# telespazio-tim/karios

Measured on AMD Instinct MI355X. Metric: Mpixels/sec (+ matched keypoints/sec), Sentinel-2 10980^2 pair, KLT + ZNCC, higher is better.
Workload: dtype u8/i32 stencils, f32 LK solve, f64 stretch + ZNCC; 1 GPU; BASELINE config 2: 4 distinct S2-sized pairs 10980x10980 u16 resident in HBM, one per step, 4 per batched submissio...; distinct_pairs_resident=4, contexts=1, klt=Laplacian k=7, maxCorners 20000, one tile, ZNCC of rows with score >= 0.4, parallelism=1 rank(s), each a stream of independent band pairs

## Files before the change

karios_amd/csrc/k_lap.hip:

```cpp
#include "k_pixel.hpp"
#include "lap_coef.hpp"

#include <algorithm>

#ifndef KM_LAPM_WAVES
#define KM_LAPM_WAVES 0
#endif
#if KM_LAPM_WAVES
#define KM_LAPM_OCC __attribute__((amdgpu_waves_per_eu(KM_LAPM_WAVES, KM_LAPM_WAVES)))
#else
#define KM_LAPM_OCC
#endif

#define LAP_TW 128
#define LAP_TH 16

template <typename T> struct stretcher {
    double mn, range;
    bool deg;
    __device__ void init(const double *mm, int img, const uint8_t *) {
        if constexpr (sizeof(T) == 1) { mn = 0; range = 1; deg = false; }
        else { mn = mm[2 * img]; const double mx = mm[2 * img + 1]; range = mx - mn; deg = !(mx > mn); }
    }
    __device__ __forceinline__ unsigned operator()(T v, const uint8_t *) const { return stretch_u8<T>(v, mn, range, deg); }
};
template <typename T> struct stretcher_i16 {
    int mn_i;
    double c1, c0;
    __device__ void init(const double *mm, int img, const uint8_t *) {
        const double mn = mm[2 * img], mx = mm[2 * img + 1];
        mn_i = (int)mn;
        if (mx > mn) { const double r = mx - mn; c1 = 255.0 / r; c0 = 0.5 / r; }
        else { c1 = 0.0; c0 = 0.0; }
    }
    __device__ __forceinline__ unsigned operator()(T v, const uint8_t *) const {
        return (unsigned)(int)__fma_rn((double)((int)v - mn_i), c1, c0);
    }
};
template <> struct stretcher<uint16_t> : stretcher_i16<uint16_t> {};
template <> struct stretcher<int16_t> : stretcher_i16<int16_t> {};

template <int R, typename T, int NIMG, bool MASK>
__global__ __launch_bounds__(256) void lap_kernel(const T *__restrict__ img0, const T *__restrict__ img1, int H, int W,
                                                  ptrdiff_t stride0, ptrdiff_t stride1, const double *__restrict__ mm,
                                                  lap_coef cf, int invert1, nodata_t nd,
                                                  uint8_t *__restrict__ out0, uint8_t *__restrict__ out1,
                                                  uint8_t *__restrict__ mask_out, unsigned *__restrict__ valid_partial)
{
    using HT = typename std::conditional<(R <= 3), short, int>::type;
    constexpr int HX = (R + 3) & ~3;
    constexpr int TWH = LAP_TW + 2 * HX;
    constexpr int THH = LAP_TH + 2 * R;
    constexpr int CPR = TWH / 4;
    constexpr int NQ = LAP_TW / 4;
    constexpr int NIT = (THH * CPR + 255) / 256;
    __shared__ uint32_t tile[NIMG][THH][CPR];
    __shared__ __attribute__((aligned(16))) HT hbuf[2][NIMG][THH][LAP_TW];
    auto &hd = hbuf[0];
    auto &hs = hbuf[1];
    const int X0 = blockIdx.x * LAP_TW, Y0 = blockIdx.y * LAP_TH;
    const int tid = threadIdx.x;
    stretcher<T> st[NIMG];
#pragma unroll
    for (int i = 0; i < NIMG; i++) st[i].init(mm, i, nullptr);
    const T *imgs[2] = {img0, img1};
    const ptrdiff_t strides[2] = {stride0, stride1};

    T v[NIT][NIMG][4];
#pragma unroll
    for (int it = 0; it < NIT; it++) {
        const int ci = it * 256 + tid;
        if (ci < THH * CPR) {
            const int row = ci / CPR, cx = ci - row * CPR;
            const int gy = km_reflect101(Y0 - R + row, H);
            const int gx0 = X0 - HX + cx * 4;
            const bool inside = gx0 >= 0 && gx0 + 3 < W;
#pragma unroll
            for (int i = 0; i < NIMG; i++) {
                const T *rowp = imgs[i] + (size_t)gy * strides[i];
                if (inside && ((((uintptr_t)(rowp + gx0)) & (4 * sizeof(T) - 1)) == 0)) {
                    if constexpr (sizeof(T) == 1) { uint32_t q = *(const uint32_t *)(rowp + gx0); __builtin_memcpy(v[it][i], &q, 4); }
                    else if constexpr (sizeof(T) == 2) { uint2 q = *(const uint2 *)(rowp + gx0); __builtin_memcpy(v[it][i], &q, 8); }
                    else { uint4 q = *(const uint4 *)(rowp + gx0); __builtin_memcpy(v[it][i], &q, 16); }
                } else {
#pragma unroll
                    for (int k = 0; k < 4; k++) v[it][i][k] = rowp[km_reflect101(gx0 + k, W)];
                }
            }
        }
    }
    unsigned cnt = 0;
#pragma unroll
    for (int it = 0; it < NIT; it++) {
        const int ci = it * 256 + tid;
        if (ci < THH * CPR) {
            const int row = ci / CPR, cx = ci - row * CPR;
            const int gx0 = X0 - HX + cx * 4;
#pragma unroll
            for (int i = 0; i < NIMG; i++) {
                uint32_t packed = 0;
#pragma unroll
                for (int k = 0; k < 4; k++) {
                    unsigned u = st[i](v[it][i][k], nullptr);
                    if (i == 1 && invert1) u = 255u - u;
                    packed |= u << (8 * k);
                }
                tile[i][row][cx] = packed;
            }
            if constexpr (MASK) {
                const int oy = Y0 - R + row;
                if (row >= R && row < R + LAP_TH && oy < H && gx0 >= X0 && gx0 < X0 + LAP_TW && gx0 < W) {
                    uint32_t mp = 0;
#pragma unroll
                    for (int k = 0; k < 4; k++) {
                        const bool ok = (gx0 + k < W) && px_valid<T>(v[it][1][k], v[it][0][k], nd);
                        mp |= (ok ? 1u : 0u) << (8 * k);
                        cnt += ok;
                    }
                    const size_t o = (size_t)oy * W + gx0;
                    if (gx0 + 3 < W && (o & 3) == 0) *(uint32_t *)(mask_out + o) = mp;
                    else {
                        for (int k = 0; k < 4 && gx0 + k < W; k++) mask_out[o + k] = (uint8_t)((mp >> (8 * k)) & 1u);
                    }
                }
            }
        }
    }
    if constexpr (MASK) {
        __shared__ unsigned s_cnt[4];
        const unsigned c64 = (unsigned)wave_sum_u64((unsigned long long)cnt);
        if ((tid & 63) == 0) s_cnt[tid >> 6] = c64;
        __syncthreads();
        if (tid == 0) valid_partial[blockIdx.y * gridDim.x + blockIdx.x] = s_cnt[0] + s_cnt[1] + s_cnt[2] + s_cnt[3];
    } else {
        __syncthreads();
    }

    uint8_t *outs[2] = {out0, out1};
    if constexpr (R <= 3) {
        typedef short short2v __attribute__((ext_vector_type(2)));
        int *hds = (int *)&hd[0][0][0];
        int kdp[NIMG][2], ksp[NIMG][2], bias[NIMG], vk[NIMG][2 * R + 1];
#pragma unroll
        for (int i = 0; i < NIMG; i++) {
            int sum = 0;
#pragma unroll
            for (int h = 0; h < 2; h++) {
                unsigned a = 0, b = 0;
#pragma unroll
                for (int k = 0; k < 4; k++) {
                    const int t = 4 * h + k;
                    const int d = t <= 2 * R ? cf.kd[i][t] : 0, sm = t <= 2 * R ? cf.ks[i][t] : 0;
                    a |= ((unsigned)d & 0xffu) << (8 * k);
                    b |= ((unsigned)sm & 0xffu) << (8 * k);
                    sum += sm;
                }
                kdp[i][h] = (int)a; ksp[i][h] = (int)b;
            }
            bias[i] = R == 4 ? 0 : 128 * sum;
#pragma unroll
            for (int t = 0; t <= 2 * R; t++) vk[i][t] = (cf.ks[i][t] & 0xffff) | (cf.kd[i][t] << 16);
        }
        for (int it = tid; it < NIMG * THH * NQ; it += 256) {
            const int i = it / (THH * NQ);
            const int rem = it - i * (THH * NQ);
            const int row = rem / NQ, q = rem - row * NQ;
            uint32_t w[4];
#pragma unroll
            for (int k = 0; k < 4; k++) w[k] = ((q + k < CPR) ? tile[i][row][q + k] : 0u) ^ 0x80808080u;
            int o4[4];
#pragma unroll
            for (int o = 0; o < 4; o++) {
                constexpr int base = HX - R;
                const int sft = (o + base) & 3, wi = (o + base) >> 2;
                const int g0 = (int)__builtin_amdgcn_alignbyte(w[wi + 1], w[wi], sft);
                const int g1 = (int)__builtin_amdgcn_alignbyte(wi + 2 < 4 ? w[wi + 2] : 0u, w[wi + 1], sft);
                const int vd = __builtin_amdgcn_sdot4(g0, kdp[i][0], __builtin_amdgcn_sdot4(g1, kdp[i][1], 0, false), false);
                const int vs = __builtin_amdgcn_sdot4(g0, ksp[i][0], __builtin_amdgcn_sdot4(g1, ksp[i][1], bias[i], false), false);
                o4[o] = (vd & 0xffff) | (vs << 16);
            }
            *(int4 *)&hds[((size_t)i * THH + row) * LAP_TW + 4 * q] = make_int4(o4[0], o4[1], o4[2], o4[3]);
        }
        __syncthreads();
        for (int it = tid; it < NIMG * (LAP_TH / 4) * NQ; it += 256) {
            const int i = it / ((LAP_TH / 4) * NQ);
            const int rem = it - i * ((LAP_TH / 4) * NQ);
            const int rg = rem / NQ, q = rem - rg * NQ;
            const int ox = X0 + 4 * q;
            if (ox >= W || Y0 + 4 * rg >= H) continue;
            int acc[4][4];
#pragma unroll
            for (int o = 0; o < 4; o++)
#pragma unroll
                for (int c2 = 0; c2 < 4; c2++) acc[o][c2] = 0;
#pragma unroll
            for (int j = 0; j < 2 * R + 4; j++) {
                const int4 a = *(const int4 *)&hds[((size_t)i * THH + 4 * rg + j) * LAP_TW + 4 * q];
                const int av[4] = {a.x, a.y, a.z, a.w};
#pragma unroll
                for (int o = 0; o < 4; o++) {
                    const int tap = j - o;
                    if (tap >= 0 && tap <= 2 * R) {
#pragma unroll
                        for (int c2 = 0; c2 < 4; c2++)
                            acc[o][c2] = __builtin_amdgcn_sdot2(__builtin_bit_cast(short2v, av[c2]), __builtin_bit_cast(short2v, vk[i][tap]),
                                                                acc[o][c2], false);
                    }
                }
            }
#pragma unroll
            for (int o = 0; o < 4; o++) {
                const int oy = Y0 + 4 * rg + o;
                if (oy >= H) break;
                uint32_t packed = 0;
#pragma unroll
                for (int k = 0; k < 4; k++) packed |= (uint32_t)min(max(acc[o][k], 0), 255) << (8 * k);
                const size_t off = (size_t)oy * W + ox;
                if (ox + 3 < W && (off & 3) == 0) *(uint32_t *)(outs[i] + off) = packed;
                else {
                    for (int k = 0; k < 4 && ox + k < W; k++) outs[i][off + k] = (uint8_t)(packed >> (8 * k));
                }
            }
        }
    } else {
        constexpr int NW = (2 * R + 4 + (HX - R) + 3) / 4;
        for (int it = tid; it < NIMG * THH * NQ; it += 256) {
            const int i = it / (THH * NQ);
            const int rem = it - i * (THH * NQ);
            const int row = rem / NQ, q = rem - row * NQ;
            uint32_t w[NW + 1];
#pragma unroll
            for (int k = 0; k < NW + 1; k++) w[k] = (q + k < CPR) ? tile[i][row][q + k] : 0u;
            int ad[4] = {0, 0, 0, 0}, as[4] = {0, 0, 0, 0};
#pragma unroll
            for (int t = 0; t < 2 * R + 4; t++) {
                const int b = t + (HX - R);
                const int pv = (int)((w[b >> 2] >> (8 * (b & 3))) & 0xffu);
#pragma unroll
                for (int o = 0; o < 4; o++) {
                    const int k = t - o;
                    if (k >= 0 && k <= 2 * R) {
                        ad[o] = mad24(cf.kd[i][k], pv, ad[o]);
                        as[o] = mad24(cf.ks[i][k], pv, as[o]);
                    }
                }
            }
            HT *pd = &hd[i][row][4 * q], *ps = &hs[i][row][4 * q];
#pragma unroll
            for (int o = 0; o < 4; o++) { pd[o] = (HT)ad[o]; ps[o] = (HT)as[o]; }
        }
        __syncthreads();
        for (int it = tid; it < NIMG * (LAP_TH / 4) * NQ; it += 256) {
            const int i = it / ((LAP_TH / 4) * NQ);
            const int rem = it - i * ((LAP_TH / 4) * NQ);
            const int rg = rem / NQ, q = rem - rg * NQ;
            const int ox = X0 + 4 * q;
            if (ox >= W || Y0 + 4 * rg >= H) continue;
            int acc[4][4];
#pragma unroll
            for (int o = 0; o < 4; o++)
#pragma unroll
                for (int c2 = 0; c2 < 4; c2++) acc[o][c2] = 0;
#pragma unroll
            for (int j = 0; j < 2 * R + 4; j++) {
                const HT *pa = &hd[i][4 * rg + j][4 * q], *pb = &hs[i][4 * rg + j][4 * q];
                int a[4], b[4];
#pragma unroll
                for (int c2 = 0; c2 < 4; c2++) { a[c2] = pa[c2]; b[c2] = pb[c2]; }
#pragma unroll
                for (int o = 0; o < 4; o++) {
                    const int tap = j - o;
                    if (tap >= 0 && tap <= 2 * R) {
                        const int ksj = cf.ks[i][tap], kdj = cf.kd[i][tap];
#pragma unroll
                        for (int c2 = 0; c2 < 4; c2++) acc[o][c2] = mad24(ksj, a[c2], mad24(kdj, b[c2], acc[o][c2]));
                    }
                }
            }
#pragma unroll
            for (int o = 0; o < 4; o++) {
                const int oy = Y0 + 4 * rg + o;
                if (oy >= H) break;
                uint32_t packed = 0;
#pragma unroll
                for (int k = 0; k < 4; k++) packed |= (uint32_t)min(max(acc[o][k], 0), 255) << (8 * k);
                const size_t off = (size_t)oy * W + ox;
                if (ox + 3 < W && (off & 3) == 0) *(uint32_t *)(outs[i] + off) = packed;
                else {
                    for (int k = 0; k < 4 && ox + k < W; k++) outs[i][off + k] = (uint8_t)(packed >> (8 * k));
                }
            }
        }
    }
}

template <typename T, int NIMG, bool MASK>
static int launch_lap(km_ctx *c, int R, const T *a, const T *b, int H, int W, ptrdiff_t sa, ptrdiff_t sb, const double *mm,
                      const lap_coef &cf, int invert1, const nodata_t &nd, uint8_t *oa, uint8_t *ob, uint8_t *mask,
                      unsigned long long *valid_out)
{
    dim3 grid((W + LAP_TW - 1) / LAP_TW, (H + LAP_TH - 1) / LAP_TH);
    unsigned *valid = nullptr;
    if (MASK) {
        valid = (unsigned *)km_ws(c, WS_PARTIAL, (size_t)grid.x * grid.y * sizeof(unsigned));
        if (!valid) return KM_E_NOMEM;
    }
#define KM_LAP_CASE(RR)                                                                                         \
    case RR:                                                                                                    \
        lap_kernel<RR, T, NIMG, MASK><<<grid, 256, 0, c->stream>>>(a, b, H, W, sa, sb, mm, cf, invert1, nd, oa, ob, \
                                                                   mask, valid);                               \
        break;
    switch (R) {
        KM_LAP_CASE(1)
        KM_LAP_CASE(2)
        KM_LAP_CASE(3)
        KM_LAP_CASE(4)
        KM_LAP_CASE(5)
    default: return km_fail(c, KM_E_UNSUPPORTED, "laplacian radius %d", R);
    }
#undef KM_LAP_CASE
    KM_LAUNCH_CHECK(c);
    return MASK ? kd_sum_u32(c, valid, grid.x * grid.y, valid_out) : KM_OK;
}

__device__ __forceinline__ int dot4_seed0(int bytes, int coef_uniform)
{
    int r;
    asm("v_dot4_i32_i8 %0, %1, %2, 0" : "=v"(r) : "v"(bytes), "s"(coef_uniform));
    return r;
}
__device__ __forceinline__ int dot4_seed(int bytes, int coef_uniform, int acc)
{
    int r;
    asm("v_dot4_i32_i8 %0, %1, %2, %3" : "=v"(r) : "v"(bytes), "s"(coef_uniform), "v"(acc));
    return r;
}
__device__ __forceinline__ int dot2_seed0(int pair, int coef_uniform)
{
    int r;
    asm("v_dot2_i32_i16 %0, %1, %2, 0" : "=v"(r) : "v"(pair), "s"(coef_uniform));
    return r;
}
__device__ __forceinline__ unsigned opaque_lane_offset(unsigned x)
{
    asm volatile("" : "+v"(x));
    return x;
}

#define LAPM_VALID_OF(R) ((R) == 5 ? 240 : 248)
#ifndef LAPM_PF
#define LAPM_PF 3
#endif

template <int R, typename T, bool MASK>
__device__ __forceinline__ void lap_march_item(const T *__restrict__ img0, const T *__restrict__ img1, int H, int W,
                                               ptrdiff_t stride0, ptrdiff_t stride1, const double *__restrict__ mm,
                                               const lap_coef &cf, int invert1, const nodata_t &nd,
                                               uint8_t *__restrict__ out0, uint8_t *__restrict__ out1,
                                               uint8_t *__restrict__ mask_out, unsigned *__restrict__ valid_partial, int nstrips,
                                               int rows_per_item, int wave_id )
{
    typedef short short2v __attribute__((ext_vector_type(2)));
    constexpr int RH = R == 5 ? 4 : R;
    constexpr int NR = 2 * RH + 1;
    constexpr int HALO = R == 5 ? 8 : 4, VALID = 256 - 2 * HALO;
    static_assert(VALID == LAPM_VALID_OF(R), "strip geometry");
    const int lane = threadIdx.x & 63;
    const int rowblock = wave_id / nstrips, strip = wave_id - rowblock * nstrips;
    stretcher<T> st[2];
    st[0].init(mm, 0, nullptr); st[1].init(mm, 1, nullptr);
    const bool shifted = (W % 4 != 0) && strip == nstrips - 1 && W >= 256;
    const int gx0 = (shifted ? W - (256 - HALO) : strip * VALID - HALO) + 4 * lane;
    const int cnt_from = shifted ? (nstrips - 1) * VALID : 0;
    const uint32_t cnt_mask = gx0 >= cnt_from ? 0xffffffffu : gx0 + 4 <= cnt_from ? 0u : (0xffffffffu << (8 * (cnt_from - gx0)));
    const unsigned ugx = (unsigned)gx0;
    const unsigned ugx_load = RH == 4 ? (unsigned)min(max(gx0 < 0 ? -gx0 - 3 : gx0 >= W ? 2 * W - 5 - gx0 : gx0, 0), W - 4) : (unsigned)min(max(gx0, 0), W - 4);
    const unsigned edge_sel = RH == 4 ? ((gx0 < 0 || gx0 >= W) ? 0x00010203u : 0x03020100u)
                                      : (gx0 < 0 ? 0x01020300u : gx0 >= W ? 0x03000102u : 0x03020100u);
    const bool col_inside = gx0 >= 0 && gx0 + 3 < W;
    const bool vec0 = col_inside && (stride0 % 4 == 0) && ((uintptr_t)img0 % (4 * sizeof(T)) == 0);
    const bool vec1 = col_inside && (stride1 % 4 == 0) && ((uintptr_t)img1 % (4 * sizeof(T)) == 0);
    int rc[4];
#pragma unroll
    for (int k = 0; k < 4; k++) rc[k] = km_reflect101(gx0 + k, W);
    const bool out_lane = lane >= HALO / 4 && lane <= 63 - HALO / 4 && gx0 < W;
    const int y0 = rowblock * rows_per_item, y1 = min(H, y0 + rows_per_item);

    constexpr int NH = RH == 4 ? 3 : 2;
    int kdp[2][NH], ksp[2][NH], bias[2], vk[2][NR];
#pragma unroll
    for (int i = 0; i < 2; i++) {
        int sum = 0;
#pragma unroll
        for (int h = 0; h < NH; h++) {
            unsigned a = 0, b = 0;
#pragma unroll
            for (int k = 0; k < 4; k++) {
                const int t = 4 * h + k;
                const int d = t < NR ? cf.kd[i][t] : 0, sm = t < NR ? cf.ks[i][t] : 0;
                a |= ((unsigned)d & 0xffu) << (8 * k);
                b |= ((unsigned)sm & 0xffu) << (8 * k);
                sum += sm;
            }
            kdp[i][h] = (int)a; ksp[i][h] = (int)b;
        }
        bias[i] = 128 * sum;
#pragma unroll
        for (int t = 0; t < NR; t++) vk[i][t] = (cf.ks[i][t] & 0xffff) | (cf.kd[i][t] << 16);
    }

    typedef unsigned short ushort2v __attribute__((ext_vector_type(2)));
    auto nodata16 = [](int has, double v) -> uint32_t {
        if (!has || v != floor(v)) return 0u;
        if constexpr (std::is_signed<T>::value) { if (v < -32768.0 || v > 32767.0) return 0u; }
        else { if (v < 0.0 || v > 65535.0) return 0u; }
        const uint32_t x = (uint32_t)(uint16_t)(int)v;
        return x | (x << 16);
    };
    const uint32_t nd16_mon = nodata16(nd.has_mon, nd.mon), nd16_ref = nodata16(nd.has_ref, nd.ref);
    (void)nd16_mon; (void)nd16_ref;
    int vbias[2];
    asm volatile("v_mov_b32 %0, %1" : "=v"(vbias[0]) : "s"(bias[0]));
    asm volatile("v_mov_b32 %0, %1" : "=v"(vbias[1]) : "s"(bias[1]));
    unsigned cnt = 0;
    uint8_t *outs[2] = {out0, out1};
    auto march = [&](auto fast_tag) {
    constexpr bool FAST = decltype(fast_tag)::value;
    auto load_raw = [&](int m, T (&v)[2][4]) {
        const int r = km_reflect101(m, H);
        const T *r0 = img0 + (size_t)r * stride0, *r1 = img1 + (size_t)r * stride1;
        const unsigned lx = opaque_lane_offset(ugx_load * (unsigned)sizeof(T));
        if (FAST) {
            __builtin_memcpy(v[0], (const char *)r0 + lx, 4 * sizeof(T));
        } else if (vec0) {
            if constexpr (sizeof(T) == 1) { uint32_t q = *(const uint32_t *)(r0 + gx0); __builtin_memcpy(v[0], &q, 4); }
            else if constexpr (sizeof(T) == 2) { uint2 q = *(const uint2 *)(r0 + gx0); __builtin_memcpy(v[0], &q, 8); }
            else { uint4 q = *(const uint4 *)(r0 + gx0); __builtin_memcpy(v[0], &q, 16); }
        } else {
#pragma unroll
            for (int k = 0; k < 4; k++) v[0][k] = r0[rc[k]];
        }
        if (FAST) {
            __builtin_memcpy(v[1], (const char *)r1 + lx, 4 * sizeof(T));
        } else if (vec1) {
            if constexpr (sizeof(T) == 1) { uint32_t q = *(const uint32_t *)(r1 + gx0); __builtin_memcpy(v[1], &q, 4); }
            else if constexpr (sizeof(T) == 2) { uint2 q = *(const uint2 *)(r1 + gx0); __builtin_memcpy(v[1], &q, 8); }
            else { uint4 q = *(const uint4 *)(r1 + gx0); __builtin_memcpy(v[1], &q, 16); }
        } else {
#pragma unroll
            for (int k = 0; k < 4; k++) v[1][k] = r1[rc[k]];
        }
    };

    int hp[2][2][4];
#pragma unroll
    for (int i = 0; i < 2; i++)
#pragma unroll
        for (int r = 0; r < 2; r++)
#pragma unroll
            for (int j = 0; j < 4; j++) hp[i][r][j] = 0;
    (void)hp;
    int ring[2][NR][4];
#pragma unroll
    for (int i = 0; i < 2; i++)
#pragma unroll
        for (int k = 0; k < NR; k++)
#pragma unroll
            for (int j = 0; j < 4; j++) ring[i][k][j] = 0;
    T nxt[LAPM_PF][2][4];
#pragma unroll
    for (int f = 0; f < LAPM_PF; f++) load_raw(min(y0 - R + f, y1 + R - 1), nxt[f]);
    for (int mbase = y0 - R; mbase < y1 + R; mbase += NR) {
#pragma unroll
        for (int k = 0; k < NR; k++) {
            const int m = mbase + k;
            if (m >= y1 + R) continue;
            T v[2][4];
#pragma unroll
            for (int i = 0; i < 2; i++)
#pragma unroll
                for (int j = 0; j < 4; j++) {
                    v[i][j] = nxt[0][i][j];
#pragma unroll
                    for (int f = 0; f + 1 < LAPM_PF; f++) nxt[f][i][j] = nxt[f + 1][i][j];
                }
            if (m + LAPM_PF < y1 + R) load_raw(m + LAPM_PF, nxt[LAPM_PF - 1]);
            if constexpr (MASK && FAST && sizeof(T) == 2) {
                if (m >= y0 && m < y1 && out_lane) {
                    uint2 qm, qr;
                    __builtin_memcpy(&qm, v[1], 8); __builtin_memcpy(&qr, v[0], 8);
                    auto nz2 = [&](uint32_t a, uint32_t b) {
                        ushort2v mn2 = __builtin_elementwise_min(
                            __builtin_elementwise_min(__builtin_bit_cast(ushort2v, a), __builtin_bit_cast(ushort2v, b)),
                            __builtin_elementwise_min(__builtin_bit_cast(ushort2v, a ^ nd16_mon), __builtin_bit_cast(ushort2v, b ^ nd16_ref)));
                        mn2 = __builtin_elementwise_min(mn2, (ushort2v)(1));
                        return __builtin_bit_cast(uint32_t, mn2);
                    };
                    const uint32_t mp = __builtin_amdgcn_perm(nz2(qm.y, qr.y), nz2(qm.x, qr.x), 0x06040200u);
                    cnt += (unsigned)__popc(mp & cnt_mask);
                    __builtin_memcpy((mask_out + (size_t)m * W) + opaque_lane_offset(ugx), &mp, 4);
                }
            } else if constexpr (MASK) {
                if (m >= y0 && m < y1 && out_lane) {
                    uint32_t mp = 0;
#pragma unroll
                    for (int j = 0; j < 4; j++) {
                        const bool ok = (gx0 + j < W) && px_valid<T>(v[1][j], v[0][j], nd);
                        mp |= (ok ? 1u : 0u) << (8 * j);
                        cnt += ok && gx0 + j >= cnt_from;
                    }
                    const size_t o = (size_t)m * W + gx0;
                    if (FAST) __builtin_memcpy(mask_out + o, &mp, 4);
                    else if (gx0 + 3 < W && (o & 3) == 0) *(uint32_t *)(mask_out + o) = mp;
                    else {
                        for (int j = 0; j < 4 && gx0 + j < W; j++) mask_out[o + j] = (uint8_t)((mp >> (8 * j)) & 1u);
                    }
                }
            }
#pragma unroll
            for (int i = 0; i < 2; i++) {
                uint32_t cw = 0;
#pragma unroll
                for (int j = 0; j < 4; j++) cw |= st[i](v[i][j], nullptr) << (8 * j);
                cw ^= (i == 1 && invert1) ? 0x7f7f7f7fu : 0x80808080u;
                if constexpr (FAST) cw = __builtin_amdgcn_perm(cw, cw, edge_sel);
                const uint32_t lw = (uint32_t)__builtin_amdgcn_update_dpp(0, (int)cw, 0x138, 0xf, 0xf, false);
                const uint32_t rw = (uint32_t)__builtin_amdgcn_update_dpp(0, (int)cw, 0x130, 0xf, 0xf, false);
#pragma unroll
                for (int o = 0; o < 4; o++) {
                    constexpr int dummy = 0; (void)dummy;
                    if constexpr (RH == 4) {
                        const int g0 = (int)__builtin_amdgcn_alignbyte(cw, lw, o), g1 = (int)__builtin_amdgcn_alignbyte(rw, cw, o),
                                  g2 = (int)__builtin_amdgcn_alignbyte(0u, rw, o);
                        const int vd = __builtin_amdgcn_sdot4(g0, kdp[i][0], __builtin_amdgcn_sdot4(g1, kdp[i][1], dot4_seed0(g2, kdp[i][2]), false), false);
                        const int vs = __builtin_amdgcn_sdot4(g0, ksp[i][0], __builtin_amdgcn_sdot4(g1, ksp[i][1], dot4_seed0(g2, ksp[i][2]), false), false);
                        ring[i][k][o] = (int)__builtin_amdgcn_perm((uint32_t)vs, (uint32_t)vd, 0x05040100u);
                        continue;
                    }
                    const int sft = 4 + o - R;
                    int g0, g1;
                    if (sft < 4) {
                        g0 = (int)__builtin_amdgcn_alignbyte(cw, lw, sft & 3);
                        g1 = (int)__builtin_amdgcn_alignbyte(rw, cw, sft & 3);
                    } else if (sft == 4) {
                        g0 = (int)cw; g1 = (int)rw;
                    } else {
                        g0 = (int)__builtin_amdgcn_alignbyte(rw, cw, (sft - 4) & 3);
                        g1 = (int)__builtin_amdgcn_alignbyte(0u, rw, (sft - 4) & 3);
                    }
                    const int vd = __builtin_amdgcn_sdot4(g0, kdp[i][0], dot4_seed0(g1, kdp[i][1]), false);
                    const int vs = __builtin_amdgcn_sdot4(g0, ksp[i][0], dot4_seed(g1, ksp[i][1], vbias[i]), false);
                    ring[i][k][o] = (int)__builtin_amdgcn_perm((uint32_t)vs, (uint32_t)vd, 0x05040100u);
                }
            }
            if constexpr (R == 5) {
                const int yy = m - RH, yo = yy - 1;
                if (yy >= y0 - 1) {
#pragma unroll
                    for (int i = 0; i < 2; i++) {
                        int a[4], h[4];
#pragma unroll
                        for (int o = 0; o < 4; o++) {
                            int acc = dot2_seed0(ring[i][(k + 1) % NR][o], vk[i][0]);
#pragma unroll
                            for (int j = 1; j < NR; j++)
                                acc = __builtin_amdgcn_sdot2(__builtin_bit_cast(short2v, ring[i][(k + 1 + j) % NR][o]),
                                                             __builtin_bit_cast(short2v, vk[i][j]), acc, false);
                            a[o] = acc;
                        }
                        uint32_t packed = 0;
                        if (cf.b3[i]) {
                            const int al = __builtin_amdgcn_update_dpp(0, a[3], 0x138, 0xf, 0xf, false);
                            const int ar = __builtin_amdgcn_update_dpp(0, a[0], 0x130, 0xf, 0xf, false);
#pragma unroll
                            for (int o = 0; o < 4; o++) h[o] = (o == 0 ? al : a[o - 1]) + 2 * a[o] + (o == 3 ? ar : a[o + 1]);
#pragma unroll
                            for (int o = 0; o < 4; o++) packed |= (uint32_t)min(max(hp[i][1][o] + 2 * hp[i][0][o] + h[o], 0), 255) << (8 * o);
                        } else {
#pragma unroll
                            for (int o = 0; o < 4; o++) { h[o] = a[o]; packed |= (uint32_t)min(max(hp[i][0][o], 0), 255) << (8 * o); }
                        }
#pragma unroll
                        for (int o = 0; o < 4; o++) { hp[i][1][o] = hp[i][0][o]; hp[i][0][o] = h[o]; }
                        if (yo >= y0 && out_lane) {
                            const size_t off = (size_t)yo * W + gx0;
                            if (FAST) __builtin_memcpy((outs[i] + (size_t)yo * W) + opaque_lane_offset(ugx), &packed, 4);
                            else if (gx0 + 3 < W && (off & 3) == 0) *(uint32_t *)(outs[i] + off) = packed;
                            else {
                                for (int j = 0; j < 4 && gx0 + j < W; j++) outs[i][off + j] = (uint8_t)(packed >> (8 * j));
                            }
                        }
                    }
                }
            } else {
            const int y = m - R;
            if (y >= y0 && out_lane) {
#pragma unroll
                for (int i = 0; i < 2; i++) {
                    uint32_t packed = 0;
#pragma unroll
                    for (int o = 0; o < 4; o++) {
                        int acc = dot2_seed0(ring[i][(k + 1) % NR][o], vk[i][0]);
#pragma unroll
                        for (int j = 1; j < NR; j++)
                            acc = __builtin_amdgcn_sdot2(__builtin_bit_cast(short2v, ring[i][(k + 1 + j) % NR][o]),
                                                         __builtin_bit_cast(short2v, vk[i][j]), acc, false);
                        packed |= (uint32_t)min(max(acc, 0), 255) << (8 * o);
                    }
                    const size_t off = (size_t)y * W + gx0;
                    if (FAST) __builtin_memcpy((outs[i] + (size_t)y * W) + opaque_lane_offset(ugx), &packed, 4);
                    else if (gx0 + 3 < W && (off & 3) == 0) *(uint32_t *)(outs[i] + off) = packed;
                    else {
                        for (int j = 0; j < 4 && gx0 + j < W; j++) outs[i][off + j] = (uint8_t)(packed >> (8 * j));
                    }
                }
            }
            }
        }
    }
    };
    const bool fast = (W % 4 == 0) || shifted || (strip * VALID - HALO + 4 * 64 <= W);
    if (fast) march(std::true_type{});
    else march(std::false_type{});
    if constexpr (MASK) {
        const unsigned c64 = (unsigned)wave_sum_u64((unsigned long long)cnt);
        if (lane == 0) valid_partial[wave_id] = c64;
    }
}

struct lapm_units_args {
    const void *img0[KM_UNITS_MAX], *img1[KM_UNITS_MAX];
    ptrdiff_t s0[KM_UNITS_MAX], s1[KM_UNITS_MAX];
    const double *mm[KM_UNITS_MAX];
    uint8_t *out0[KM_UNITS_MAX], *out1[KM_UNITS_MAX], *mask[KM_UNITS_MAX];
    unsigned *valid[KM_UNITS_MAX];
    int H[KM_UNITS_MAX], W[KM_UNITS_MAX], nstrips[KM_UNITS_MAX];
    int item0[KM_UNITS_MAX + 1];
    int n, rows;
};
template <int R, typename T, bool MASK>
__global__ __launch_bounds__(256) KM_LAPM_OCC void lap_march_units_kernel(lapm_units_args U, lap_coef cf, int invert1, nodata_t nd)
{
    const int total = U.item0[U.n];
    unsigned tile;
    if (!km_xcd_tile((unsigned)(total + 3) / 4u, tile)) return;
    const int wave_lin = (int)tile * 4 + __builtin_amdgcn_readfirstlane(threadIdx.x >> 6);
    if (wave_lin >= total) return;
    int u = 0;
    while (u + 1 < U.n && wave_lin >= U.item0[u + 1]) u++;
    lap_march_item<R, T, MASK>((const T *)U.img0[u], (const T *)U.img1[u], U.H[u], U.W[u], U.s0[u], U.s1[u], U.mm[u], cf, invert1, nd, U.out0[u], U.out1[u],
                               U.mask[u], U.valid[u], U.nstrips[u], U.rows, wave_lin - U.item0[u]);
}

template <typename T, bool MASK>
static const void *lapm_kernel(int R)
{
    return R == 1 ? (const void *)lap_march_units_kernel<1, T, MASK> : R == 2 ? (const void *)lap_march_units_kernel<2, T, MASK>
         : R == 3 ? (const void *)lap_march_units_kernel<3, T, MASK> : R == 4 ? (const void *)lap_march_units_kernel<4, T, MASK>
         : (const void *)lap_march_units_kernel<5, T, MASK>;
}

static void lapm_items(km_ctx *c, int R, const void *fn, lapm_units_args &A)
{
    int wg_per_cu = 0;
    if (hipOccupancyMaxActiveBlocksPerMultiprocessor(&wg_per_cu, fn, 256, 0) != hipSuccess || wg_per_cu < 1) wg_per_cu = 4;
    int rows = km_pick_rows_units(A.H, A.nstrips, A.n, 2 * R, (long)c->n_cu * 4 * wg_per_cu, 32, 160);
    if (const char *e = km_dev_env("KARIOS_HIP_LAP_ROWS")) { const int v = atoi(e); if (v >= 8 && v <= 4096) rows = v; }
    A.rows = rows;
    A.item0[0] = 0;
    for (int u = 0; u < A.n; u++) A.item0[u + 1] = A.item0[u] + A.nstrips[u] * ((A.H[u] + rows - 1) / rows);
}

static int lapm_launch(km_ctx *c, const void *fn, const lapm_units_args &A, const lap_coef &cf, int invert1, const nodata_t &nd)
{
    void *args[] = {(void *)&A, (void *)&cf, (void *)&invert1, (void *)&nd};
    KM_HIP(c, hipLaunchKernel(fn, dim3(km_xcd_grid((unsigned)(A.item0[A.n] + 3) / 4u)), dim3(256), args, 0, c->stream));
    return KM_OK;
}

template <typename T, bool MASK>
static int launch_lap_march(km_ctx *c, int R, const T *a, const T *b, int H, int W, ptrdiff_t sa, ptrdiff_t sb, const double *mm,
                            const lap_coef &cf, int invert1, const nodata_t &nd, uint8_t *oa, uint8_t *ob,
                            uint8_t *mask, unsigned long long *valid_out, km_valid_job *defer)
{
    lapm_units_args A;
    A.n = 1;
    A.img0[0] = a; A.img1[0] = b; A.s0[0] = sa; A.s1[0] = sb; A.mm[0] = mm;
    A.out0[0] = oa; A.out1[0] = ob; A.mask[0] = mask; A.valid[0] = nullptr;
    A.H[0] = H; A.W[0] = W; A.nstrips[0] = (W + LAPM_VALID_OF(R) - 1) / LAPM_VALID_OF(R);
    const void *fn = lapm_kernel<T, MASK>(R);
    lapm_items(c, R, fn, A);
    const unsigned nitems = (unsigned)A.item0[1];
    if (MASK) {
        A.valid[0] = (unsigned *)km_ws(c, WS_LAP_VALID, ((size_t)nitems + 4) * sizeof(unsigned));
        if (!A.valid[0]) return KM_E_NOMEM;
    }
    if (int rc = lapm_launch(c, fn, A, cf, invert1, nd)) return rc;
    if (MASK) {
        if (defer) {
            defer->partial = A.valid[0]; defer->n = nitems; defer->out = valid_out;
        } else if (int rc = kd_sum_u32(c, A.valid[0], nitems, valid_out)) return rc;
    }
    return KM_OK;
}

int kd_run_valid_sum(km_ctx *c, km_valid_job *job)
{
    if (!job->partial) return KM_OK;
    const km_valid_job j = *job;
    *job = km_valid_job();
    return kd_sum_u32(c, j.partial, j.n, j.out);
}

__global__ __launch_bounds__(64) void valid_sum_units_kernel(km_valid_units J)
{
    const unsigned *partial = J.partial[blockIdx.x];
    const unsigned n = J.n_partial[blockIdx.x];
    unsigned long long s = 0;
    for (unsigned i = threadIdx.x; i < n; i += 64) s += partial[i];
    s = wave_sum_u64(s);
    if (threadIdx.x == 0) *J.out[blockIdx.x] = s;
}

int kd_valid_sum_units(km_ctx *c, const km_valid_units &J)
{
    if (J.n <= 0) return KM_OK;
    valid_sum_units_kernel<<<J.n, 64, 0, c->stream>>>(J);
    KM_LAUNCH_CHECK(c);
    return KM_OK;
}

struct mask_units_args {
    const uint8_t *src[KM_UNITS_MAX];
    uint8_t *dst[KM_UNITS_MAX];
    ptrdiff_t stride[KM_UNITS_MAX];
    unsigned *partial[KM_UNITS_MAX];
    int H[KM_UNITS_MAX], W[KM_UNITS_MAX];
};
__global__ __launch_bounds__(256) void mask_pack_units_kernel(mask_units_args A)
{
    const int u = blockIdx.y, H = A.H[u], W = A.W[u];
    const uint8_t *__restrict__ src = A.src[u];
    uint8_t *__restrict__ dst = A.dst[u];
    const ptrdiff_t stride = A.stride[u];
    unsigned cnt = 0;
    for (int y = blockIdx.x; y < H; y += gridDim.x) {
        const uint8_t *r = src + (size_t)y * stride;
        uint8_t *w = dst + (size_t)y * W;
        for (int x = 16 * threadIdx.x; x < W; x += 16 * 256) {
            if (x + 16 <= W) {
                uint4 q;
                __builtin_memcpy(&q, r + x, 16);
                __builtin_memcpy(w + x, &q, 16);
                const uint32_t d[4] = {q.x, q.y, q.z, q.w};
#pragma unroll
                for (int k = 0; k < 4; k++) cnt += (unsigned)__popc(((d[k] | ((d[k] & 0x7f7f7f7fu) + 0x7f7f7f7fu)) & 0x80808080u));
            } else {
                for (int k = x; k < W; k++) { const uint8_t b = r[k]; w[k] = b; cnt += b != 0; }
            }
        }
    }
    const unsigned long long s = wave_sum_u64((unsigned long long)cnt);
    __shared__ unsigned sh[4];
    if ((threadIdx.x & 63) == 0) sh[threadIdx.x >> 6] = (unsigned)s;
    __syncthreads();
    if (threadIdx.x == 0) A.partial[u][blockIdx.x] = sh[0] + sh[1] + sh[2] + sh[3];
}

template <typename T>
static int launch_lap_march_units(km_ctx *c, int R, const km_units &U, const lap_coef &cf, int invert1, const nodata_t &nd, km_valid_units *job)
{
    lapm_units_args A;
    A.n = U.n;
    for (int u = 0; u < U.n; u++) {
        A.img0[u] = U.ref[u]; A.img1[u] = U.mon[u]; A.s0[u] = U.sref[u]; A.s1[u] = U.smon[u]; A.mm[u] = U.mm[u];
        A.out0[u] = U.lap_ref[u]; A.out1[u] = U.lap_mon[u]; A.mask[u] = U.mask[u];
        A.H[u] = U.H[u]; A.W[u] = U.W[u]; A.nstrips[u] = (U.W[u] + LAPM_VALID_OF(R) - 1) / LAPM_VALID_OF(R);
    }
    lapm_items(c, R, lapm_kernel<T, true>(R), A);
    const int total = A.item0[U.n];
    const int mask_wgs = 256;
    const size_t n_partial = U.has_user_mask ? (size_t)mask_wgs * U.n : (size_t)total + 4 * KM_UNITS_MAX;
    unsigned *valid = (unsigned *)km_ws(c, WS_LAP_VALID, n_partial * sizeof(unsigned));
    if (!valid) return KM_E_NOMEM;
    job->n = U.n;
    if (U.has_user_mask) {
        mask_units_args M;
        for (int u = 0; u < U.n; u++) {
            M.src[u] = U.user_mask[u]; M.dst[u] = U.mask[u]; M.stride[u] = U.user_smask[u]; M.H[u] = U.H[u]; M.W[u] = U.W[u];
            M.partial[u] = valid + (size_t)mask_wgs * u;
            A.valid[u] = nullptr;
            job->partial[u] = M.partial[u]; job->n_partial[u] = (unsigned)mask_wgs; job->out[u] = &U.sc[u]->valid;
        }
        mask_pack_units_kernel<<<dim3(mask_wgs, U.n), 256, 0, c->stream>>>(M);
        KM_LAUNCH_CHECK(c);
        return lapm_launch(c, lapm_kernel<T, false>(R), A, cf, invert1, nd);
    }
    for (int u = 0; u < U.n; u++) {
        A.valid[u] = valid + A.item0[u];
        job->partial[u] = A.valid[u]; job->n_partial[u] = (unsigned)(A.item0[u + 1] - A.item0[u]); job->out[u] = &U.sc[u]->valid;
    }
    return lapm_launch(c, lapm_kernel<T, true>(R), A, cf, invert1, nd);
}

enum lap_form { LAP_NOT_COVERED = 0, LAP_GENERAL, LAP_MARCH };
struct lap_plan {
    int R = 0;
    lap_coef cf;
    lap_form form = LAP_NOT_COVERED;
};
static lap_plan lap_make_plan(int ksize_ref, int ksize_mon, int min_W, int min_H)
{
    lap_plan p;
    if (!km_lap_ksize_ok(ksize_ref) || !km_lap_ksize_ok(ksize_mon)) return p;
    const int ks[2] = {ksize_ref, ksize_mon};
    p.R = std::max(std::max(ksize_ref, ksize_mon) / 2, 1);
    const int edge = p.R == 5 ? 16 : 8;
    const bool march = min_W >= edge && min_H >= edge, march5 = march && p.R == 5;
    for (int i = 0; i < 2; i++) {
        p.cf.b3[i] = march5 && ks[i] == 11;
        if (!fill_coef(p.cf.b3[i] ? 9 : ks[i], march5 ? 4 : p.R, p.cf.kd[i], p.cf.ks[i])) return p;
    }
    p.form = march ? LAP_MARCH : LAP_GENERAL;
    return p;
}

int kd_stretch_laplacian_units(km_ctx *c, const km_units &U, int ksize_ref, int ksize_mon, int invert_mon, const double *nodata_ref,
                               const double *nodata_mon, km_valid_units *job)
{
    const lap_plan p = lap_make_plan(ksize_ref, ksize_mon, *std::min_element(U.W, U.W + U.n), *std::min_element(U.H, U.H + U.n));
    if (p.form == LAP_NOT_COVERED) return km_fail(c, KM_E_UNSUPPORTED, "Laplacian ksize ref=%d mon=%d (supported: 1,3,5,7,9,11)", ksize_ref, ksize_mon);
    if (p.form != LAP_MARCH) return KM_E_UNSUPPORTED;
    const nodata_t nd = make_nodata(nodata_mon, nodata_ref);
    return km_with_pixel_type(c, U.dtype, "stretch_laplacian: bad dtype %d",
                              [&](auto t) { return launch_lap_march_units<decltype(t)>(c, p.R, U, p.cf, invert_mon, nd, job); });
}

int kd_laplacian_u8(km_ctx *c, const uint8_t *d_src, int H, int W, int ksize, uint8_t *d_dst)
{
    const lap_plan p = lap_make_plan(ksize, ksize, 0, 0);
    if (p.form == LAP_NOT_COVERED) return km_fail(c, KM_E_UNSUPPORTED, "Laplacian ksize %d (supported: 1,3,5,7,9,11)", ksize);
    return launch_lap<uint8_t, 1, false>(c, p.R, d_src, d_src, H, W, W, W, nullptr, p.cf, 0, make_nodata(nullptr, nullptr), d_dst, nullptr, nullptr,
                                         nullptr);
}

int kd_stretch_laplacian_pair(km_ctx *c, const void *d_ref, const void *d_mon, int dtype, int H, int W, ptrdiff_t sref,
                              ptrdiff_t smon, const double *d_mm, int ksize_ref, int ksize_mon, int invert_mon,
                              const double *nodata_ref, const double *nodata_mon, uint8_t *d_lap_ref, uint8_t *d_lap_mon,
                              uint8_t *d_mask_out, unsigned long long *d_valid, km_valid_job *defer)
{
    const lap_plan p = lap_make_plan(ksize_ref, ksize_mon, W, H);
    if (p.form == LAP_NOT_COVERED) return km_fail(c, KM_E_UNSUPPORTED, "Laplacian ksize ref=%d mon=%d (supported: 1,3,5,7,9,11)", ksize_ref, ksize_mon);
    const nodata_t nd = make_nodata(nodata_mon, nodata_ref);
    return km_with_pixel_type(c, dtype, "stretch_laplacian: bad dtype %d", [&](auto t) {
        using T = decltype(t);
        const T *ref = (const T *)d_ref, *mon = (const T *)d_mon;
        if (p.form == LAP_MARCH)
            return d_mask_out ? launch_lap_march<T, true>(c, p.R, ref, mon, H, W, sref, smon, d_mm, p.cf, invert_mon, nd, d_lap_ref, d_lap_mon, d_mask_out, d_valid, defer)
                              : launch_lap_march<T, false>(c, p.R, ref, mon, H, W, sref, smon, d_mm, p.cf, invert_mon, nd, d_lap_ref, d_lap_mon, nullptr, nullptr, nullptr);
        return d_mask_out ? launch_lap<T, 2, true>(c, p.R, ref, mon, H, W, sref, smon, d_mm, p.cf, invert_mon, nd, d_lap_ref, d_lap_mon, d_mask_out, d_valid)
                          : launch_lap<T, 2, false>(c, p.R, ref, mon, H, W, sref, smon, d_mm, p.cf, invert_mon, nd, d_lap_ref, d_lap_mon, nullptr, nullptr);
    });
}
```

Before: 153,700 Mpx/s.

## Split Laplacian march into warmup and branch-free interior loop with buffer stores

Restructures the row-march loop of the fused Laplacian/mask kernel into three phases: a guarded warmup, a branch-free interior phase, and a guarded tail. The interior phase uses a rotating slot buffer with pointer-increment loads, raw buffer stores whose out-of-range lanes are handled by the buffer descriptor bounds, and sched barriers between rows. This removes per-row boundary checks and 64-bit address arithmetic from the hot loop. It also swaps update_dpp for mov_dpp with bound_ctrl. The cost is more code and register pressure, plus a risk that the descriptor bounds or lane masking are subtly wrong.

```diff
diff --git a/karios_amd/csrc/k_lap.hip b/karios_amd/csrc/k_lap.hip
--- a/karios_amd/csrc/k_lap.hip
+++ b/karios_amd/csrc/k_lap.hip
@@ -346,6 +346,12 @@
     asm volatile("" : "+v"(x));
     return x;
 }
+__device__ __forceinline__ void reopaque_lane_offset(unsigned &x) { asm volatile("" : "+v"(x)); }
+template <class F, int... I> __device__ __forceinline__ void lapm_for_impl(F &&f, std::integer_sequence<int, I...>)
+{
+    (f(std::integral_constant<int, I>{}), ...);
+}
+template <int N, class F> __device__ __forceinline__ void lapm_for(F &&f) { lapm_for_impl(f, std::make_integer_sequence<int, N>{}); }
 
 #define LAPM_VALID_OF(R) ((R) == 5 ? 240 : 248)
 #ifndef LAPM_PF
@@ -467,26 +473,16 @@
         for (int k = 0; k < NR; k++)
 #pragma unroll
             for (int j = 0; j < 4; j++) ring[i][k][j] = 0;
-    T nxt[LAPM_PF][2][4];
-#pragma unroll
-    for (int f = 0; f < LAPM_PF; f++) load_raw(min(y0 - R + f, y1 + R - 1), nxt[f]);
-    for (int mbase = y0 - R; mbase < y1 + R; mbase += NR) {
-#pragma unroll
-        for (int k = 0; k < NR; k++) {
-            const int m = mbase + k;
-            if (m >= y1 + R) continue;
-            T v[2][4];
-#pragma unroll
-            for (int i = 0; i < 2; i++)
-#pragma unroll
-                for (int j = 0; j < 4; j++) {
-                    v[i][j] = nxt[0][i][j];
-#pragma unroll
-                    for (int f = 0; f + 1 < LAPM_PF; f++) nxt[f][i][j] = nxt[f + 1][i][j];
-                }
-            if (m + LAPM_PF < y1 + R) load_raw(m + LAPM_PF, nxt[LAPM_PF - 1]);
+    __amdgpu_buffer_rsrc_t rs_m = __builtin_amdgcn_make_buffer_rsrc((void *)nullptr, 0, 0, 0x00020000), rs_o0 = rs_m, rs_o1 = rs_m;
+    unsigned srow = 0;
+    const unsigned ux = out_lane ? ugx : 0x80000000u;
+    const uint32_t cnt_mask_in = out_lane ? cnt_mask : 0u;
+    (void)srow; (void)ux; (void)cnt_mask_in;
+    auto row_step = [&](auto k_tag, auto in_tag, int m, const T (&v)[2][4]) {
+            constexpr int k = decltype(k_tag)::value;
+            constexpr bool IN = decltype(in_tag)::value;
             if constexpr (MASK && FAST && sizeof(T) == 2) {
-                if (m >= y0 && m < y1 && out_lane) {
+                if (IN || (m >= y0 && m < y1 && out_lane)) {
                     uint2 qm, qr;
                     __builtin_memcpy(&qm, v[1], 8); __builtin_memcpy(&qr, v[0], 8);
                     auto nz2 = [&](uint32_t a, uint32_t b) {
@@ -497,20 +493,29 @@
                         return __builtin_bit_cast(uint32_t, mn2);
                     };
                     const uint32_t mp = __builtin_amdgcn_perm(nz2(qm.y, qr.y), nz2(qm.x, qr.x), 0x06040200u);
-                    cnt += (unsigned)__popc(mp & cnt_mask);
-                    __builtin_memcpy((mask_out + (size_t)m * W) + opaque_lane_offset(ugx), &mp, 4);
+                    if constexpr (IN) {
+                        cnt += (unsigned)__popc(mp & cnt_mask_in);
+                        __builtin_amdgcn_raw_buffer_store_b32(mp, rs_m, ux, srow, 0);
+                    } else {
+                        cnt += (unsigned)__popc(mp & cnt_mask);
+                        __builtin_memcpy((mask_out + (size_t)m * W) + opaque_lane_offset(ugx), &mp, 4);
+                    }
                 }
             } else if constexpr (MASK) {
-                if (m >= y0 && m < y1 && out_lane) {
+                if (IN || (m >= y0 && m < y1 && out_lane)) {
                     uint32_t mp = 0;
 #pragma unroll
                     for (int j = 0; j < 4; j++) {
                         const bool ok = (gx0 + j < W) && px_valid<T>(v[1][j], v[0][j], nd);
                         mp |= (ok ? 1u : 0u) << (8 * j);
-                        cnt += ok && gx0 + j >= cnt_from;
+                        if constexpr (!IN) cnt += ok && gx0 + j >= cnt_from;
                     }
                     const size_t o = (size_t)m * W + gx0;
-                    if (FAST) __builtin_memcpy(mask_out + o, &mp, 4);
+                    (void)o;
+                    if constexpr (IN) {
+                        cnt += (unsigned)__popc(mp & cnt_mask_in);
+                        __builtin_amdgcn_raw_buffer_store_b32(mp, rs_m, ux, srow, 0);
+                    } else if (FAST) __builtin_memcpy(mask_out + o, &mp, 4);
                     else if (gx0 + 3 < W && (o & 3) == 0) *(uint32_t *)(mask_out + o) = mp;
                     else {
                         for (int j = 0; j < 4 && gx0 + j < W; j++) mask_out[o + j] = (uint8_t)((mp >> (8 * j)) & 1u);
@@ -524,8 +529,8 @@
                 for (int j = 0; j < 4; j++) cw |= st[i](v[i][j], nullptr) << (8 * j);
                 cw ^= (i == 1 && invert1) ? 0x7f7f7f7fu : 0x80808080u;
                 if constexpr (FAST) cw = __builtin_amdgcn_perm(cw, cw, edge_sel);
-                const uint32_t lw = (uint32_t)__builtin_amdgcn_update_dpp(0, (int)cw, 0x138, 0xf, 0xf, false);
-                const uint32_t rw = (uint32_t)__builtin_amdgcn_update_dpp(0, (int)cw, 0x130, 0xf, 0xf, false);
+                const uint32_t lw = (uint32_t)__builtin_amdgcn_mov_dpp((int)cw, 0x138, 0xf, 0xf, true);
+                const uint32_t rw = (uint32_t)__builtin_amdgcn_mov_dpp((int)cw, 0x130, 0xf, 0xf, true);
 #pragma unroll
                 for (int o = 0; o < 4; o++) {
                     constexpr int dummy = 0; (void)dummy;
@@ -555,7 +560,7 @@
             }
             if constexpr (R == 5) {
                 const int yy = m - RH, yo = yy - 1;
-                if (yy >= y0 - 1) {
+                if (IN || yy >= y0 - 1) {
 #pragma unroll
                     for (int i = 0; i < 2; i++) {
                         int a[4], h[4];
@@ -570,8 +575,8 @@
                         }
                         uint32_t packed = 0;
                         if (cf.b3[i]) {
-                            const int al = __builtin_amdgcn_update_dpp(0, a[3], 0x138, 0xf, 0xf, false);
-                            const int ar = __builtin_amdgcn_update_dpp(0, a[0], 0x130, 0xf, 0xf, false);
+                            const int al = __builtin_amdgcn_mov_dpp(a[3], 0x138, 0xf, 0xf, true);
+                            const int ar = __builtin_amdgcn_mov_dpp(a[0], 0x130, 0xf, 0xf, true);
 #pragma unroll
                             for (int o = 0; o < 4; o++) h[o] = (o == 0 ? al : a[o - 1]) + 2 * a[o] + (o == 3 ? ar : a[o + 1]);
 #pragma unroll
@@ -582,9 +587,11 @@
                         }
 #pragma unroll
                         for (int o = 0; o < 4; o++) { hp[i][1][o] = hp[i][0][o]; hp[i][0][o] = h[o]; }
-                        if (yo >= y0 && out_lane) {
+                        if (IN || (yo >= y0 && out_lane)) {
                             const size_t off = (size_t)yo * W + gx0;
-                            if (FAST) __builtin_memcpy((outs[i] + (size_t)yo * W) + opaque_lane_offset(ugx), &packed, 4);
+                            (void)off;
+                            if constexpr (IN) __builtin_amdgcn_raw_buffer_store_b32(packed, i == 0 ? rs_o0 : rs_o1, ux, srow, 0);
+                            else if (FAST) __builtin_memcpy((outs[i] + (size_t)yo * W) + opaque_lane_offset(ugx), &packed, 4);
                             else if (gx0 + 3 < W && (off & 3) == 0) *(uint32_t *)(outs[i] + off) = packed;
                             else {
                                 for (int j = 0; j < 4 && gx0 + j < W; j++) outs[i][off + j] = (uint8_t)(packed >> (8 * j));
@@ -594,7 +601,7 @@
                 }
             } else {
             const int y = m - R;
-            if (y >= y0 && out_lane) {
+            if (IN || (y >= y0 && out_lane)) {
 #pragma unroll
                 for (int i = 0; i < 2; i++) {
                     uint32_t packed = 0;
@@ -608,7 +615,9 @@
                         packed |= (uint32_t)min(max(acc, 0), 255) << (8 * o);
                     }
                     const size_t off = (size_t)y * W + gx0;
-                    if (FAST) __builtin_memcpy((outs[i] + (size_t)y * W) + opaque_lane_offset(ugx), &packed, 4);
+                    (void)off;
+                    if constexpr (IN) __builtin_amdgcn_raw_buffer_store_b32(packed, i == 0 ? rs_o0 : rs_o1, ux, srow, 0);
+                    else if (FAST) __builtin_memcpy((outs[i] + (size_t)y * W) + opaque_lane_offset(ugx), &packed, 4);
                     else if (gx0 + 3 < W && (off & 3) == 0) *(uint32_t *)(outs[i] + off) = packed;
                     else {
                         for (int j = 0; j < 4 && gx0 + j < W; j++) outs[i][off + j] = (uint8_t)(packed >> (8 * j));
@@ -616,7 +625,70 @@
                 }
             }
             }
-        }
+    };
+
+    constexpr int DEPTH = (R == 5 && sizeof(T) == 4 && LAPM_PF > 2) ? 2 : LAPM_PF;
+    constexpr int PF = DEPTH < NR ? DEPTH : NR - 1;
+    constexpr int WARM = (2 * R + NR - 1) / NR * NR;
+    const int m_end = y1 + R;
+    int mbase = y0 - R;
+    int n_in = 0;
+    if constexpr (FAST) n_in = (min(y1, min(H, m_end) - PF) - (mbase + WARM)) / NR;
+    int m_stop = n_in > 0 ? mbase + WARM : m_end;
+    for (;;) {
+        {
+            T nxt[DEPTH][2][4];
+#pragma unroll
+            for (int f = 0; f < DEPTH; f++) load_raw(min(mbase + f, m_end - 1), nxt[f]);
+            for (; mbase < m_stop; mbase += NR) {
+                lapm_for<NR>([&](auto k_tag) {
+                    const int m = mbase + decltype(k_tag)::value;
+                    if (m >= m_end) return;
+                    T v[2][4];
+#pragma unroll
+                    for (int i = 0; i < 2; i++)
+#pragma unroll
+                        for (int j = 0; j < 4; j++) {
+                            v[i][j] = nxt[0][i][j];
+#pragma unroll
+                            for (int f = 0; f + 1 < DEPTH; f++) nxt[f][i][j] = nxt[f + 1][i][j];
+                        }
+                    if (m + DEPTH < m_end) load_raw(m + DEPTH, nxt[DEPTH - 1]);
+                    row_step(k_tag, std::false_type{}, m, v);
+                });
+            }
+        }
+        if (mbase >= m_end) break;
+        if constexpr (FAST) {
+            const ptrdiff_t sb0 = stride0 * (ptrdiff_t)sizeof(T), sb1 = stride1 * (ptrdiff_t)sizeof(T);
+            const char *p0 = (const char *)img0 + (ptrdiff_t)mbase * sb0, *p1 = (const char *)img1 + (ptrdiff_t)mbase * sb1;
+            unsigned lx = ugx_load * (unsigned)sizeof(T);
+            auto load_next = [&](T (&v)[2][4]) {
+                reopaque_lane_offset(lx);
+                __builtin_memcpy(v[0], p0 + lx, 4 * sizeof(T));
+                __builtin_memcpy(v[1], p1 + lx, 4 * sizeof(T));
+                p0 += sb0; p1 += sb1;
+            };
+            T slot[NR][2][4];
+#pragma unroll
+            for (int f = 0; f < PF; f++) load_next(slot[f]);
+            const int span = n_in * NR * W;
+            if constexpr (MASK) rs_m = __builtin_amdgcn_make_buffer_rsrc((void *)(mask_out + (size_t)mbase * W), 0, span, 0x00020000);
+            rs_o0 = __builtin_amdgcn_make_buffer_rsrc((void *)(out0 + (size_t)(mbase - R) * W), 0, span, 0x00020000);
+            rs_o1 = __builtin_amdgcn_make_buffer_rsrc((void *)(out1 + (size_t)(mbase - R) * W), 0, span, 0x00020000);
+            srow = 0;
+            for (int t = 0; t < n_in; t++) {
+                lapm_for<NR>([&](auto k_tag) {
+                    constexpr int k = decltype(k_tag)::value;
+                    load_next(slot[(k + PF) % NR]);
+                    row_step(k_tag, std::true_type{}, mbase + k, slot[k]);
+                    srow += (unsigned)W;
+                    __builtin_amdgcn_sched_barrier(0);
+                });
+                mbase += NR;
+            }
+        }
+        m_stop = m_end;
     }
     };
     const bool fast = (W % 4 == 0) || shifted || (strip * VALID - HALO + 4 * 64 <= W);
```

Result: faster. 163,100 Mpx/s (median of 6 runs) (+6.1%).
